# DanielaCourel/smoothed_particle_hydrodynamics

Measured on AMD Instinct MI355X. Metric: Mparticle-steps/sec (whole node), dam-break, higher is better.
Workload: dtype f32

## Files before the change

include/sph_hip.h:

```cpp
#ifndef SPH_HIP_H
#define SPH_HIP_H

#include <stddef.h>
#include <stdint.h>

#ifdef __cplusplus
extern "C" {
#endif

#define SPH_HIP_ABI_VERSION 7
#define SPH_HIP_ABI_DIAGNOSTIC 0x4000
int sph_hip_abi_version(void);

typedef enum sph_hip_status {
   SPH_HIP_OK = 0,
   SPH_HIP_ERR_INVALID = -1,
   SPH_HIP_ERR_DEVICE = -2,
   SPH_HIP_ERR_CAPACITY = -3,
   SPH_HIP_ERR_NO_DEVICE = -4,
   SPH_HIP_ERR_EXCHANGE = -5
} sph_hip_status;

typedef enum sph_hip_mode {
   SPH_HIP_MODE_REF = 0,
// ... 42 lines not shown
#define SPH_HIP_MIN_EXAMINE_COUNT 4
int sph_hip_create(sph_hip_context** out, const sph_hip_params* params, int capacity, int mode,
                   int device);
void sph_hip_destroy(sph_hip_context* ctx);

const char* sph_hip_last_error(const sph_hip_context* ctx);

int sph_hip_set_params(sph_hip_context* ctx, const sph_hip_params* params);
int sph_hip_get_params(const sph_hip_context* ctx, sph_hip_params* out);

#define SPH_HIP_ARITH_EXACT 0
#define SPH_HIP_ARITH_FAST 1
int sph_hip_set_arithmetic(sph_hip_context* ctx, int arithmetic);
int sph_hip_get_arithmetic(const sph_hip_context* ctx);


int sph_hip_upload(sph_hip_context* ctx, int n, const float* pos, const float* vel,
                   const float* mass);

int sph_hip_download(sph_hip_context* ctx, float* pos, float* vel, float* density, float* acc,
                     int32_t* neighbor_count);

int sph_hip_download_async(sph_hip_context* ctx, float* pos, float* vel, float* density, float* acc,
                           int32_t* neighbor_count, int32_t* voxel_counts, int* started);
int sph_hip_download_done(sph_hip_context* ctx, int wait);
int sph_hip_host_register(void* ptr, size_t bytes);
int sph_hip_host_unregister(void* ptr);

int sph_hip_particle_count(const sph_hip_context* ctx);


int sph_hip_step(sph_hip_context* ctx);
int sph_hip_run(sph_hip_context* ctx, int steps);

int sph_hip_voxelize(sph_hip_context* ctx);
int sph_hip_find_neighbors(sph_hip_context* ctx);
int sph_hip_compute_density(sph_hip_context* ctx);
int sph_hip_compute_acceleration(sph_hip_context* ctx);
int sph_hip_integrate(sph_hip_context* ctx);

int sph_hip_synchronize(sph_hip_context* ctx);


int sph_hip_get_timings(sph_hip_context* ctx, float ms[6]);
int sph_hip_get_phase_totals(sph_hip_context* ctx, double ms[6], int32_t* steps);
int sph_hip_reset_timings(sph_hip_context* ctx);
#define SPH_HIP_TIMING_OFF 0
#define SPH_HIP_TIMING_SUMS 1
#define SPH_HIP_TIMING_PHASES 2
int sph_hip_set_timing(sph_hip_context* ctx, int level);
int sph_hip_set_timing_stride(sph_hip_context* ctx, int every);

int sph_hip_get_tile_stats(sph_hip_context* ctx, int32_t out[20]);

int sph_hip_get_energy(sph_hip_context* ctx, float* kinetic, float* potential);

int sph_hip_get_neighbor_stats(sph_hip_context* ctx, int32_t* avg, int32_t* max, int32_t* min);

int sph_hip_download_voxels(sph_hip_context* ctx, int32_t* coords_xyz, int32_t* ids);
int sph_hip_download_grid_counts(sph_hip_context* ctx, int32_t* counts);
int sph_hip_download_neighbor_lists(sph_hip_context* ctx, uint32_t* neighbors, float* distances);


int sph_hip_sample_points(sph_hip_context* ctx, int n, const float* xyz,
                          float* density, float* velocity_xyz, int32_t* count);
int sph_hip_sample_lattice(sph_hip_context* ctx, const float origin[3], const float spacing[3],
                           const int32_t dims[3], float* density, float* velocity_xyz, int32_t* count);

#define SPH_HIP_SURFACE_NORMALS  1
#define SPH_HIP_SURFACE_VELOCITY 2
int sph_hip_extract_surface(sph_hip_context* ctx, const float origin[3], const float spacing[3],
                            const int32_t dims[3], float iso, int flags, int32_t counts[2]);
int sph_hip_download_surface(sph_hip_context* ctx, float* vertices_xyz, float* normals_xyz,
                             float* velocity_xyz, int32_t* triangles);

typedef struct sph_hip_camera {
   float eye[3];
   float forward[3];
   float right[3];
   float up[3];
} sph_hip_camera;

typedef struct sph_hip_render_params {
   float box_lo[3], box_hi[3];
   float step;
   float iso;
   int32_t refine;
   float grad_step;
   float light[3];
   float albedo[3], ambient, diffuse;
   uint8_t background[4];
   int32_t max_samples;
} sph_hip_render_params;

#define SPH_HIP_RENDER_VELOCITY 1
int sph_hip_render(sph_hip_context* ctx, const sph_hip_camera* cam, const sph_hip_render_params* rp,
                   int width, int height, int flags, uint8_t* rgba, float* depth,
                   float* normal_xyz, float* velocity_xyz, int32_t* first_inside);

typedef struct sph_hip_scene_params {
   float albedo[3];
   float ambient, diffuse;
} sph_hip_scene_params;

int sph_hip_render_scene(sph_hip_context* ctx, const sph_hip_camera* cam, const sph_hip_render_params* rp,
                         const sph_hip_scene_params* sp, const float* solid_albedo_rgb ,
// ... 173 lines not shown
```

smoothed_particle_hydrodynamics_amd/csrc/full_tiled.h:

```cpp
#pragma once

#include "launch_policy.h"
#include "tile_layout.h"
#include "common_kernels.h"
#include "full_kernels.h"
#include "neighbor_lists.h"
#include "slab_kernels.h"

#if defined(SPH_ABLATE) && !defined(SPH_DIAGNOSTIC_BUILD)
#error "SPH_ABLATE is for diagnostic builds only: add -DSPH_DIAGNOSTIC_BUILD (tools/build_variant.sh does)"
#endif

#ifdef SPH_TRIPCOUNT
#ifndef SPH_DIAGNOSTIC_BUILD
#error "SPH_TRIPCOUNT is for diagnostic builds only: add -DSPH_DIAGNOSTIC_BUILD"
#endif
enum {
   TRIP_D_WAVES = 0, TRIP_D_CHUNKS_W, TRIP_D_TEST8_W, TRIP_D_TEST8_L, TRIP_D_SLOTS_L, TRIP_D_POPS_W,
   TRIP_D_POPS_L, TRIP_D_POPLOOPS_W, TRIP_D_SUMTRIPS_W, TRIP_D_SUMSLOTS_W, TRIP_D_LISTED_L, TRIP_D_LANES_L,
   TRIP_A_WAVES = 16, TRIP_A_PTRIPS_W, TRIP_A_CNT_L, TRIP_A_VTRIPS_W, TRIP_A_NV_L, TRIP_A_LANES_L,
   TRIP_COUNT = 32
};
__device__ unsigned long long g_trip[TRIP_COUNT];
struct TripCounters {
// ... 38 lines not shown

constexpr int TILE_BATCH = 8;
#define DENSITY_TILE_BYTES 12
#define ACCEL_TILE_BYTES 16
constexpr int DENSITY_BLOCKS = 6 * 256 / TILE_THREADS;
constexpr int ACCEL_BLOCKS = TILE_THREADS == 256 ? 5 : 2;
constexpr int APPEND_POPS = 4;
constexpr int VISC_UNROLL = 4;

typedef float __attribute__((ext_vector_type(2))) f32x2;
typedef float __attribute__((ext_vector_type(4))) f32x4;

__device__ __forceinline__ f32x4 lds_read4(const float* base, int i)
{
   return *reinterpret_cast<const f32x4*>(__builtin_assume_aligned(base + i, 16));
}

struct TileLds {
   float* x;
   float* y;
   float* z;
};

extern __shared__ __attribute__((aligned(16))) float tile_lds_dynamic[];

__device__ __forceinline__ void
tile_desc(int tile, int ntiles, const uint32_t* __restrict__ perm, const uint32_t* __restrict__ key,
          const uint32_t* __restrict__ cell_start, const int32_t* __restrict__ meta, CellGrid g,
          TileDesc* __restrict__ desc, const TileCaps& caps, int32_t* __restrict__ stats,
          uint32_t* __restrict__ giveup_density, uint32_t* __restrict__ giveup_accel)
{
   const int begin = meta[META_SUM_BEGIN], end = meta[META_SUM_END];
   const int p0 = begin + tile * TILE_THREADS;
   int most = -1;
   if (tile < ntiles && p0 < end) {
      const int plast = min(p0 + TILE_THREADS - 1, end - 1);
      const int c_first = (int)key[perm[p0]];
      const int c_last = (int)key[perm[plast]];
      TileDesc d;
      int G[9], len[9];
#pragma unroll
      for (int k = 0; k < 9; k++) {
         const int off = ((k / 3 - 1) * g.ny + (k % 3 - 1)) * g.nx;
         int lo = c_first + off - 1, hi = c_last + off + 1;
         lo = lo < 0 ? 0 : lo;
         hi = hi > g.ncells - 1 ? g.ncells - 1 : hi;
         G[k] = 0;
         len[k] = 0;
         if (hi >= lo) {
            G[k] = (int)cell_start[lo];
            len[k] = (int)cell_start[hi + 1] - G[k];
         }
      }
      tile_layout_chain(G, len, d);
      const int run = d.total;
      desc[tile] = d;
      most = run;
   }
   const bool lead = (threadIdx.x & (SPH_WAVE - 1)) == 0;
#pragma unroll
   for (int c = 0; c < TILE_CANDS; c++) {
      const int over = __popcll(__ballot(c < caps.n_cand && most > caps.cand[c]));
      if (lead && over) atomicAdd(&stats[TSTAT_OVER + c], over);
   }
   int wave_most = most;
#pragma unroll
   for (int o = SPH_WAVE / 2; o > 0; o >>= 1) wave_most = max(wave_most, __shfl_xor(wave_most, o));
   if (lead && wave_most > stats[TSTAT_MAX]) atomicMax(&stats[TSTAT_MAX], wave_most);
   if (most > caps.cap_density) giveup_density[atomicAdd(&stats[TSTAT_GIVEUP_DENSITY], 1)] = (uint32_t)tile;
   if (most > caps.cap_density || most > caps.cap_accel)
      giveup_accel[atomicAdd(&stats[TSTAT_GIVEUP_ACCEL], 1)] = (uint32_t)tile;
}

__global__ void __launch_bounds__(256)
k_rank_gather_tile_desc(int desc_blocks, int ntiles, const uint32_t* __restrict__ perm,
                        const uint32_t* __restrict__ key, const uint32_t* __restrict__ cell_start,
                        const int32_t* __restrict__ meta, CellGrid g,
                        const float4* __restrict__ posm_in, const float4* __restrict__ velp_in,
                        float4* __restrict__ posm_out, float4* __restrict__ velp_out,
                        TileDesc* __restrict__ desc, TileCaps caps, int32_t* __restrict__ stats,
                        uint32_t* __restrict__ giveup_density, uint32_t* __restrict__ giveup_accel,
                        uint32_t* __restrict__ remap)
{
   if ((int)blockIdx.x < desc_blocks) {
      tile_desc(blockIdx.x * blockDim.x + threadIdx.x, ntiles, perm, key, cell_start, meta, g, desc,
                caps, stats, giveup_density, giveup_accel);
      return;
   }
   __shared__ uint32_t lds_id[256];
   rank_gather((blockIdx.x - desc_blocks) * blockDim.x + threadIdx.x,
               (blockIdx.x - desc_blocks) * blockDim.x, lds_id, perm, key, cell_start, meta,
               g.ncells, posm_in, velp_in, posm_out, velp_out, remap);
}

__device__ __forceinline__ void tile_desc_load(const TileDesc* __restrict__ desc, int wg, TileDesc& sd)
{
   const int tid = threadIdx.x;
   if (tid < (int)(sizeof(TileDesc) / sizeof(int)))
      reinterpret_cast<int*>(&sd)[tid] = reinterpret_cast<const int*>(&desc[wg])[tid];
   __syncthreads();
}

__device__ __forceinline__ int xcd_workgroup(int block, int nblocks)
{
   const int q = nblocks / 8, r = nblocks % 8, x = block % 8;
   return (x < r ? x * (q + 1) : r * (q + 1) + (x - r) * q) + block / 8;
}
// ... 593 lines not shown
            to_right = near_right;
         } else if (near_left || near_right) {
            atomicOr(&fs.meta[META_ERRORS], 8);
         }
      }
      if (fs.zone.have_left) {
         const int s = msg_reserve(&fs.left->header[0], to_left);
         if (to_left) {
            if (s < fs.msg_capacity) {
               fs.left->rec[2 * s] = x;
               fs.left->rec[2 * s + 1] = v;
            } else {
               atomicOr(&fs.meta[META_ERRORS], 2);
            }
         }
      }
      if (fs.zone.have_right) {
         const int s = msg_reserve(&fs.right->header[0], to_right);
         if (to_right) {
            if (s < fs.msg_capacity) {
               fs.right->rec[2 * s] = x;
               fs.right->rec[2 * s + 1] = v;
            } else {
               atomicOr(&fs.meta[META_ERRORS], 2);
            }
         }
      }
   }
   __shared__ double s_ke[TILE_THREADS / SPH_WAVE], s_pe[TILE_THREADS / SPH_WAVE];
#pragma unroll
   for (int d = SPH_WAVE / 2; d > 0; d >>= 1) {
      ke += __shfl_down(ke, d);
      pe += __shfl_down(pe, d);
   }
   const int lane = threadIdx.x & (SPH_WAVE - 1), w = threadIdx.x / SPH_WAVE;
   if (lane == 0) {
      s_ke[w] = ke;
      s_pe[w] = pe;
   }
   __syncthreads();
   if (threadIdx.x == 0) {
      double sa = 0.0, sb = 0.0;
#pragma unroll
      for (int q = 0; q < TILE_THREADS / SPH_WAVE; q++) {
         sa += s_ke[q];
         sb += s_pe[q];
      }
      fs.epart[2 * wg_index + 0] = sa;
      fs.epart[2 * wg_index + 1] = sb;
   }
   __syncthreads();
}

template <bool UNIT_SCALE, bool UNIFORM_MASS, bool WIDE, bool FAST>
__device__ __forceinline__ float4
accel_from_lists(int p, int cnt, const ListReader& lr, const TileDesc& d,
                 const float4* __restrict__ posm, const float4* __restrict__ velB,
                 const float* __restrict__ rho, const float* __restrict__ auxc, const PairConsts& k)
{
   const float4 pi = posm[p];
   AccelState s;
   accel_begin(k, s, pi, velB[p], rho[p]);
   const bool in_range = accel_operands_in_range(k);
   int first_v = 0;
   if (FAST) first_v = visc_first(cnt, s.visc_scale);
   if constexpr (FAST) {
      const int lastb = cnt > 0 ? (cnt - 1) >> 3 : 0;
      uint4 blk = lr.block(0);
      for (int j0 = 0; j0 < cnt; j0 += 8) {
         uint32_t entry[8];
         list_block_entries(blk, entry);
         blk = lr.block(min((j0 >> 3) + 1, lastb));
         float4 pj[8];
         float cj[8];
#pragma unroll
         for (int u = 0; u < 8; u++) {
            const uint32_t e = j0 + u < cnt ? entry[u] : entry[0];
            const int q = ListEntry<WIDE>::tile(e) - ListEntry<WIDE>::shift(d, e);
            pj[u] = posm[q];
            cj[u] = auxc[q];
         }
#pragma unroll
         for (int u = 0; u < 8; u++) {
            if (j0 + u < cnt) {
               float dx, dy, dz;
               float dd = sqrt_rn(dist2(pi.x, pi.y, pi.z, pj[u].x, pj[u].y, pj[u].z, dx, dy, dz));
               if (!UNIT_SCALE) dd *= k.sim_scale;
               accel_pair_fast_pressure<UNIT_SCALE>(k, s, dx, dy, dz, dd, cj[u]);
            }
         }
      }
      for (int j0 = first_v; j0 < cnt; j0 += VISC_UNROLL) {
         float4 pj[VISC_UNROLL], vj[VISC_UNROLL];
#pragma unroll
         for (int u = 0; u < VISC_UNROLL; u++) {
            const uint32_t e = lr.entry((uint32_t)min(j0 + u, cnt - 1));
            const int q = ListEntry<WIDE>::tile(e) - ListEntry<WIDE>::shift(d, e);
            pj[u] = posm[q];
            vj[u] = velB[q];
         }
#pragma unroll
         for (int u = 0; u < VISC_UNROLL; u++) {
            if (j0 + u < cnt) {
               float dx, dy, dz;
               float dd = sqrt_rn(dist2(pi.x, pi.y, pi.z, pj[u].x, pj[u].y, pj[u].z, dx, dy, dz));
               if (!UNIT_SCALE) dd *= k.sim_scale;
// ... 24 lines not shown
            float dx, dy, dz;
            const float d2 = dist2(pi.x, pi.y, pi.z, pj[u].x, pj[u].y, pj[u].z, dx, dy, dz);
            float dd = sqrt_rn(d2);
            if (!UNIT_SCALE) dd *= k.sim_scale;
            if (FAST) {
               accel_pair_fast_pressure<UNIT_SCALE>(k, s, dx, dy, dz, dd, cj[u]);
               if (j0 + u >= first_v) accel_pair_fast_viscous(k, s, dd, vj[u].x, vj[u].y, vj[u].z, vj[u].w);
            } else {
               accel_pair<UNIT_SCALE>(k, s, dx, dy, dz, dd, UNIFORM_MASS ? pi.w : pj[u].w, vj[u].x, vj[u].y,
                                      vj[u].z, vj[u].w, cj[u], in_range);
            }
         }
      }
   }
   if (FAST) accel_fast_finish(k, s);
   return accel_end<UNIT_SCALE>(k, s);
}

template <bool UNIT_SCALE, bool UNIFORM_MASS, bool WIDE, bool FAST>
__global__ void __launch_bounds__(TILE_THREADS, ACCEL_BLOCKS)
k_full_accel_lists(const float4* __restrict__ posm, const float4* __restrict__ velB,
                   const float* __restrict__ rho, const float* __restrict__ auxc,
                   const int32_t* __restrict__ ncount, const uint32_t* __restrict__ cell_start,
                   const int32_t* __restrict__ meta, CellGrid g, PairConsts k,
                   float4* __restrict__ acc, const TileDesc* __restrict__ desc,
                   const uint32_t* __restrict__ nlist, const uint32_t* __restrict__ nlist_overflow,
                   int tile_cap, const int32_t* __restrict__ tile_stats,
                   const uint32_t* __restrict__ giveup, int part, int list_cap,
                   int* __restrict__ tile_feedback, FusedStep fs, int tile_cap_density)
{
   PHASE_BEGIN();
   __shared__ AccelLds L;
   float4* xyzc = reinterpret_cast<float4*>(tile_lds_dynamic);
   constexpr int BATCH = TILE_BATCH;

   const int begin = meta[META_SUM_BEGIN], end = meta[META_SUM_END];
   const int ob = meta[META_OWN_BEGIN], oe = meta[META_OWN_END];
   const int tid = threadIdx.x;
   const int wgs = tile_stats[TSTAT_BLOCKS];
   const int mapped = accel_part_workgroup(part, blockIdx.x, wgs, begin, meta);
   const int wg = mapped < 0 ? 0 : mapped;
   const int p0 = begin + wg * TILE_THREADS;
   if (blockIdx.x == 0 && tid == 0) {
      tile_feedback[TSTAT_NO_LIST] = tile_stats[TSTAT_NO_LIST];
      if (fs.slab && part == 1) {
         if (fs.left) fs.left->header[1] = fs.msg_capacity;
         if (fs.right) fs.right->header[1] = fs.msg_capacity;
      }
   }
   const bool own = mapped >= 0 && !(p0 >= end || p0 + TILE_THREADS <= ob || p0 >= oe) &&
                    accel_part_has(part, p0, meta);
   const uint32_t gave_up = own ? nlist_overflow[wg] : LISTS_NONE;
   int desc_word = 0;
   if (tid < (int)(sizeof(TileDesc) / sizeof(int))) desc_word = reinterpret_cast<const int*>(&desc[wg])[tid];
   if ((int)blockIdx.x < tile_stats[TSTAT_GIVEUP_ACCEL]) {
      const int g0 = begin + (int)giveup[blockIdx.x] * TILE_THREADS;
      const int gp = g0 + tid;
      const bool mine = gp < end && gp >= ob && gp < oe && accel_part_has(part, g0, meta);
      const int gwg = (int)giveup[blockIdx.x];
      const uint32_t glists = nlist_overflow[gwg];
      if (glists != LISTS_NONE) {
         tile_desc_load(desc, gwg, L.desc);
         if (mine) {
            const int gcnt = ncount[gp];
            const ListReader glr(nlist, gwg, list_cap, tid);
            if (glists == LISTS_SOME && gcnt > 0 && glr.no_list())
               accel_untiled<UNIT_SCALE, FAST>(gp, posm, velB, rho, auxc, cell_start, g, k, acc, ncount);
            else
               acc[gp] = accel_from_lists<UNIT_SCALE, UNIFORM_MASS, WIDE, FAST>(gp, gcnt, glr, L.desc, posm, velB,
                                                                                rho, auxc, k);
         }
         __syncthreads();
      } else if (mine) {
         accel_untiled<UNIT_SCALE, FAST>(gp, posm, velB, rho, auxc, cell_start, g, k, acc, ncount);
      }
      if (fs.on && accel_part_has(part, g0, meta)) {
         float4 gx = make_float4(0.f, 0.f, 0.f, 0.f), ga = gx;
         if (mine) {
            gx = posm[gp];
            ga = acc[gp];
         }
         fused_integrate<UNIT_SCALE>(fs, k, g, gp, mine, gx, ga, (int)giveup[blockIdx.x]);
      }
   }
   if (gave_up == LISTS_NONE) return;
   if (tid < (int)(sizeof(TileDesc) / sizeof(int))) reinterpret_cast<int*>(&L.desc)[tid] = desc_word;
   __syncthreads();
   PHASE_MARK(16);
   const int total = L.desc.total;
   if (total > tile_cap || total > tile_cap_density) return;
   int B[9], D[9];
#pragma unroll
   for (int kk = 0; kk < 9; kk++) {
      B[kk] = L.desc.B[kk];
      D[kk] = L.desc.D[kk];
   }
   float4 buf[BATCH];
   float cbuf[BATCH];
#if defined(SPH_ABLATE) && SPH_ABLATE == 23
#pragma unroll
   for (int r = 0; r < BATCH; r++) {
      buf[r] = make_float4(0.f, 0.f, 0.f, 0.f);
      cbuf[r] = 0.f;
   }
   const int filled = 0;
#else
#pragma unroll
   for (int r = 0; r < BATCH; r++) {
      const int idx = min(tid + r * TILE_THREADS, total - 1);
      int d = D[0];
#pragma unroll
      for (int kk = 1; kk < 9; kk++) d = (idx >= B[kk]) ? D[kk] : d;
      buf[r] = posm[idx - d];
      cbuf[r] = auxc[idx - d];
   }
   const int filled = total;
#endif

   const int col = tid;
   const int p = p0 + col;
   const bool live = p < end && p >= ob && p < oe;
   float4 pi = make_float4(0.f, 0.f, 0.f, 0.f);
   float4 vi = pi;
   float rho_i = 0.0f;
   int cnt = 0;
   if (live) {
      pi = posm[p];
      vi = velB[p];
      rho_i = rho[p];
      cnt = ncount[p];
   }

   const ListReader lr(nlist, wg, list_cap, col);
   uint32_t entry[LIST_BLOCK_ENTRIES];
   uint4 next_blk = lr.block(0);

#pragma unroll
   for (int r = 0; r < BATCH; r++) {
      const int idx = tid + r * TILE_THREADS;
      if (idx < filled) xyzc[idx] = make_float4(buf[r].x, buf[r].y, buf[r].z, cbuf[r]);
   }

   AccelState s;
   int first_v = 0;
   bool no_list = false;
   float4 vpre[VISC_UNROLL];
   int tpre[VISC_UNROLL], nvp = 0;
   uint32_t ev[VISC_UNROLL];
   if constexpr (FAST) {
      static_assert(VISC_UNROLL == 4, "list_entries_from takes four entries");
      accel_begin(k, s, pi, vi, rho_i);
      first_v = visc_first(cnt, s.visc_scale);
      const int lcnt = cnt <= list_cap ? cnt : 0;
      const int fv = lcnt > 0 ? first_v : 0;
      const int lb = lcnt > 0 ? (lcnt - 1) >> 3 : 0;
      const int fb = fv >> 3;
      const uint4 blk_a = lr.block(fb), blk_b = lr.block(min(fb + 1, lb));
      if (gave_up == LISTS_SOME && cnt > 0) no_list = next_blk.x == NLIST_NO_LIST;
      nvp = no_list ? 0 : lcnt - fv;
      list_entries_from(blk_a, blk_b, (uint32_t)(fv & 7), ev);
   }

   for (int base = BATCH * TILE_THREADS; base < filled; base += BATCH * TILE_THREADS) {
#pragma unroll
      for (int r = 0; r < BATCH; r++) {
         const int idx = min(base + tid + r * TILE_THREADS, filled - 1);
         int d = D[0];
#pragma unroll
         for (int kk = 1; kk < 9; kk++) d = (idx >= B[kk]) ? D[kk] : d;
         buf[r] = posm[idx - d];
         cbuf[r] = auxc[idx - d];
      }
#pragma unroll
      for (int r = 0; r < BATCH; r++) {
         const int idx = base + tid + r * TILE_THREADS;
         if (idx < filled) xyzc[idx] = make_float4(buf[r].x, buf[r].y, buf[r].z, cbuf[r]);
      }
   }
   if constexpr (FAST) {
#pragma unroll
      for (int u = 0; u < VISC_UNROLL; u++) {
         tpre[u] = ListEntry<WIDE>::tile(ev[u]);
         vpre[u] = make_float4(0.f, 0.f, 0.f, 0.f);
         if (u < nvp) vpre[u] = velB[tpre[u] - ListEntry<WIDE>::shift(L.desc, ev[u])];
      }
   }
   __syncthreads();

   PHASE_MARK(17);
   if constexpr (!FAST) accel_begin(k, s, pi, vi, rho_i);
   const bool in_range = accel_operands_in_range(k);
   if constexpr (!FAST) {
      if (gave_up == LISTS_SOME && cnt > 0) no_list = next_blk.x == NLIST_NO_LIST;
   }
   if (no_list) cnt = 0;
#if defined(SPH_ABLATE) && (SPH_ABLATE == 21 || SPH_ABLATE == 23)
   cnt = 0;
#endif
   const int lastb = cnt > 0 ? (cnt - 1) >> 3 : 0;
   if constexpr (FAST) {
      TRIP(TripCounters trips; trips.wave(TRIP_A_WAVES - 16, true); trips.lane(TRIP_A_CNT_L - 16, (unsigned)cnt);
           trips.lane(TRIP_A_LANES_L - 16, live ? 1u : 0u); trips.lane(TRIP_A_NV_L - 16, (unsigned)(cnt - first_v));)
      const int nv = cnt - first_v;
      if (__any(0 < nv)) {
#pragma unroll
         for (int u = 0; u < VISC_UNROLL; u++) {
            if (u < nv) {
               const float4 pj = xyzc[tpre[u]];
               float dx, dy, dz;
               float d = sqrt_rn(dist2(pi.x, pi.y, pi.z, pj.x, pj.y, pj.z, dx, dy, dz));
               if (!UNIT_SCALE) d *= k.sim_scale;
               accel_pair_fast_viscous(k, s, d, vpre[u].x, vpre[u].y, vpre[u].z, vpre[u].w);
            }
         }
      }
      for (int m0 = VISC_UNROLL; __any(m0 < nv); m0 += VISC_UNROLL) {
         float4 vj[VISC_UNROLL];
         int tj[VISC_UNROLL];
#pragma unroll
         for (int u = 0; u < VISC_UNROLL; u++) {
            const int j = min(first_v + m0 + u, cnt > 0 ? cnt - 1 : 0);
            const uint32_t e = lr.entry((uint32_t)j);
            tj[u] = ListEntry<WIDE>::tile(e);
            vj[u] = make_float4(0.f, 0.f, 0.f, 0.f);
            if (m0 + u < nv) vj[u] = velB[tj[u] - ListEntry<WIDE>::shift(L.desc, e)];
// ... 133 lines not shown
```

smoothed_particle_hydrodynamics_amd/csrc/sph_hip.hip:

```cpp

#include "slab_comm.h"

#ifndef M_PI
#define M_PI 3.14159265358979323846
#endif

namespace {

__global__ void k_selftest_sqrt(unsigned long long* __restrict__ out)
{
   unsigned long long bad = 0;
   uint32_t first = 0xffffffffu, last = 0u;
   const uint32_t stride = gridDim.x * blockDim.x;
   for (uint64_t b = blockIdx.x * blockDim.x + threadIdx.x; b <= 0x7f7fffffull; b += stride) {
      const float x = __uint_as_float((uint32_t)b);
      const float want = sqrtf(x), got = sqrt_rn(x);
      if (__float_as_uint(want) != __float_as_uint(got)) {
         bad++;
         first = min(first, (uint32_t)b);
         last = max(last, (uint32_t)b);
      }
   }
   if (bad) {
      atomicAdd(&out[0], bad);
// ... 1495 lines not shown

int sph_hip_reset_timings(sph_hip_context* ctx)
{
   if (!ctx) return SPH_HIP_ERR_INVALID;
   ctx->ev_steps = 0;
   return SPH_HIP_OK;
}

int sph_hip_get_phase_totals(sph_hip_context* ctx, double ms[6], int32_t* steps)
{
   int rc = check_ctx(ctx);
   if (rc) return rc;
   if (!ms || !steps) return SPH_HIP_ERR_INVALID;
   const long long have = ctx->ev_steps < EV_RING ? ctx->ev_steps : EV_RING;
   for (int k = 0; k < 6; k++) ms[k] = 0.0;
   for (long long s = ctx->ev_steps - have; s < ctx->ev_steps; s++) {
      float one[6];
      if ((rc = read_phases(ctx, ctx->ev[s % EV_RING], one))) return rc;
      for (int k = 0; k < 6; k++) ms[k] += (double)one[k];
   }
   *steps = (int32_t)have;
   return SPH_HIP_OK;
}

int sph_hip_get_energy(sph_hip_context* ctx, float* kinetic, float* potential)
{
   int rc = check_ctx(ctx);
   if (rc) return rc;
   double e[2] = {0.0, 0.0};
   if (ctx->energy_blocks > 0) {
      hipLaunchKernelGGL(k_energy_total, dim3(1), dim3(RED_THREADS), 0, ctx->stream,
                         ctx->epart + 2, ctx->energy_blocks, ctx->epart);
      SPH_TRY(hipGetLastError());
   }
   SPH_TRY(hipMemcpyAsync(e, ctx->epart, sizeof(e), hipMemcpyDeviceToHost, ctx->stream));
   SPH_TRY(hipStreamSynchronize(ctx->stream));
   if (kinetic) *kinetic = (float)e[0];
   if (potential) *potential = (float)e[1];
   return SPH_HIP_OK;
}

int sph_hip_get_tile_stats(sph_hip_context* ctx, int32_t out[20])
{
   int rc = check_ctx(ctx);
   if (rc) return rc;
   if (!out || !ctx->tile_feedback) return SPH_HIP_ERR_INVALID;
   SPH_TRY(hipStreamSynchronize(ctx->stream));
   for (int i = 0; i < 16; i++) out[i] = ctx->tile_feedback[i];
   out[16] = ctx->caps.cap_density;
   out[17] = ctx->caps.cap_accel;
   out[18] = ctx->caps.wide;
   out[19] = ctx->list_cap;
   return SPH_HIP_OK;
}

int sph_hip_get_neighbor_stats(sph_hip_context* ctx, int32_t* avg, int32_t* mx, int32_t* mn)
{
   int rc = check_ctx(ctx);
   if (rc) return rc;
   if ((rc = owned_count(ctx, nullptr))) return rc;
   const int n = ctx->n_owned;
   if (n == 0) return SPH_HIP_ERR_INVALID;
   const int32_t init[4] = {0, 0, -1, 34};
   SPH_TRY(hipMemcpyAsync(ctx->stats, init, sizeof(init), hipMemcpyHostToDevice, ctx->stream));
   int blocks = div_up(n, RED_THREADS);
   if (blocks > 1024) blocks = 1024;
   hipLaunchKernelGGL(k_neighbor_stats, dim3(blocks), dim3(RED_THREADS), 0, ctx->stream,
                      ctx->ncount, ctx->meta, ctx->stats);
   SPH_TRY(hipGetLastError());
   int32_t out[4];
   SPH_TRY(hipMemcpyAsync(out, ctx->stats, sizeof(out), hipMemcpyDeviceToHost, ctx->stream));
   SPH_TRY(hipStreamSynchronize(ctx->stream));
   const long long sum = ((long long)(uint32_t)out[1] << 32) | (uint32_t)out[0];
   if (avg) *avg = (int32_t)(sum / n);
   if (mx) *mx = out[2];
   if (mn) *mn = out[3];
   return SPH_HIP_OK;
}

int sph_hip_download_voxels(sph_hip_context* ctx, int32_t* coords_xyz, int32_t* ids)
{
   int rc = check_ctx(ctx);
   if (rc) return rc;
   if (ctx->mode != SPH_HIP_MODE_REF) {
      ctx->err = "sph_hip_download_voxels: REF-mode contexts only";
      return SPH_HIP_ERR_INVALID;
   }
   const int n = ctx->n_owned;
   if (coords_xyz)
      SPH_TRY(hipMemcpyAsync(coords_xyz, ctx->vox, sizeof(int32_t) * 3 * n, hipMemcpyDeviceToHost,
                             ctx->stream));
   if (ids)
      SPH_TRY(hipMemcpyAsync(ids, ctx->key, sizeof(int32_t) * n, hipMemcpyDeviceToHost, ctx->stream));
   SPH_TRY(hipStreamSynchronize(ctx->stream));
   return SPH_HIP_OK;
}

int sph_hip_download_grid_counts(sph_hip_context* ctx, int32_t* counts)
{
   int rc = check_ctx(ctx);
   if (rc) return rc;
   if (!counts) return SPH_HIP_ERR_INVALID;
   const int nc = ctx->grid.ncells;
   uint32_t* tmp = (uint32_t*)malloc(sizeof(uint32_t) * ((size_t)nc + 1));
   if (!tmp) return SPH_HIP_ERR_INVALID;
   hipError_t e = hipMemcpyAsync(tmp, ctx->cell_start, sizeof(uint32_t) * ((size_t)nc + 1),
// ... 578 lines not shown
```

smoothed_particle_hydrodynamics_amd/csrc/tile_layout.h:

```cpp
#pragma once

#include <stdint.h>

#include "launch_policy.h"

#ifdef __HIPCC__
#define TILE_HD __host__ __device__ inline __attribute__((always_inline))
#else
#define TILE_HD inline
#endif

#define TILE_SEGMENTS 9
#define TILE_EACH_BOUNDARY(X) X(1, 0) X(2, 1) X(3, 2) X(4, 3) X(5, 4) X(6, 5) X(7, 6) X(8, 7)
#define TILE_WORDS(k, prev) const int B##k = B[k], D##k = D[k];
#define TILE_LOCALS const int D0 = D[0]; TILE_EACH_BOUNDARY(TILE_WORDS)

struct TileDesc {
   int D[9];
   int B[9];
   int total;
   int pad;
};

TILE_HD void tile_layout_chain(const int (&G)[TILE_SEGMENTS], const int (&len)[TILE_SEGMENTS], TileDesc& d)
{
   int run = 0, chain_end = -1, chain_d = 0;
#ifdef __HIPCC__
#pragma unroll
#endif
   for (int k = 0; k < TILE_SEGMENTS; k++) {
      d.B[k] = run;
      if (len[k] == 0) {
         d.D[k] = run - G[k];
      } else if (G[k] <= chain_end) {
         const int seg_end = G[k] + len[k];
         d.D[k] = chain_d;
         if (seg_end > chain_end) {
            run += seg_end - chain_end;
            chain_end = seg_end;
         }
      } else {
         d.D[k] = chain_d = run - G[k];
         run += len[k];
         chain_end = G[k] + len[k];
      }
   }
   d.total = run;
   d.pad = 0;
}

TILE_HD int tile_shift_at(const int (&B)[TILE_SEGMENTS], const int (&D)[TILE_SEGMENTS], int t)
{
   TILE_LOCALS
   int d = D0;
#define TILE_STEP(k, prev) d = (t >= B##k) ? D##k : d;
   TILE_EACH_BOUNDARY(TILE_STEP)
#undef TILE_STEP
   return d;
}

TILE_HD uint32_t tile_pass_boundaries(const int (&B)[TILE_SEGMENTS], const int (&D)[TILE_SEGMENTS], int lo, int hi)
{
   TILE_LOCALS
   uint32_t m = 0;
#define TILE_STEP(k, prev) m |= ((B##k > lo) & (B##k < hi) & (D##k != D##prev)) ? 1u << k : 0u;
   TILE_EACH_BOUNDARY(TILE_STEP)
#undef TILE_STEP
   return m;
}

TILE_HD uint64_t tile_pass_mask(const int (&B)[TILE_SEGMENTS], const int (&D)[TILE_SEGMENTS], int total)
{
   TILE_LOCALS
   uint64_t m = 0;
#define TILE_STEP(k, prev)                                                                          \
   m |= ((B##k > 0) & (B##k < total) & (B##k % TILE_THREADS != 0) & (D##k != D##prev))             \
           ? 1ull << (B##k / TILE_THREADS < 63 ? B##k / TILE_THREADS : 63) : 0ull;
   TILE_EACH_BOUNDARY(TILE_STEP)
#undef TILE_STEP
   return m;
}
TILE_HD bool tile_pass_has_boundary(uint64_t mask, int q)
{
   return (mask >> (q < 63 ? q : 63)) & 1u;
}

struct TilePassPlan {
   int first, end;
   int shift;
   int n;
   int B[TILE_SEGMENTS - 1];
   int D[TILE_SEGMENTS - 1];
};
TILE_HD void tile_pass_plan(const TileDesc& d, int q, TilePassPlan& p)
{
   p.first = q * TILE_THREADS;
   p.end = p.first + TILE_THREADS < d.total ? p.first + TILE_THREADS : d.total;
   if (p.end < p.first) p.end = p.first;
   p.shift = tile_shift_at(d.B, d.D, p.first);
   p.n = 0;
   if (!tile_pass_has_boundary(tile_pass_mask(d.B, d.D, d.total), q)) return;
   const uint32_t m = tile_pass_boundaries(d.B, d.D, p.first, p.end);
   for (int k = 1; k < TILE_SEGMENTS; k++)
      if (m >> k & 1u) {
         p.B[p.n] = d.B[k];
         p.D[p.n] = d.D[k];
         p.n++;
      }
}
```

smoothed_particle_hydrodynamics_amd/lib.py:

```python
import collections
import ctypes as C
import os

from .build import library_path

MODE_REF = 0
MODE_FULL = 1
MODE_FULL_FAST = 2
ARITH_EXACT, ARITH_FAST = 0, 1
ABI_DIAGNOSTIC = 0x4000
TIMING_OFF, TIMING_SUMS, TIMING_PHASES = 0, 1, 2


class SphHipError(RuntimeError):
    pass


class SphParams(C.Structure):

    _fields_ = [
        ("cells_x", C.c_int32), ("cells_y", C.c_int32), ("cells_z", C.c_int32),
        ("cell_size", C.c_float),
        ("max_x", C.c_float), ("max_y", C.c_float), ("max_z", C.c_float),
        ("h", C.c_float), ("h2", C.c_float), ("hscaled", C.c_float), ("hscaled2", C.c_float),
# ... 35 lines not shown

    _fields_ = [
        ("box_lo", C.c_float * 3), ("box_hi", C.c_float * 3),
        ("step", C.c_float), ("iso", C.c_float), ("refine", C.c_int32), ("grad_step", C.c_float),
        ("light", C.c_float * 3), ("albedo", C.c_float * 3), ("ambient", C.c_float), ("diffuse", C.c_float),
        ("background", C.c_uint8 * 4), ("max_samples", C.c_int32),
    ]


class SphSceneParams(C.Structure):

    _fields_ = [("albedo", C.c_float * 3), ("ambient", C.c_float), ("diffuse", C.c_float)]


from . import obstacles as _obstacles
from .obstacles import (SphBody, SphBodyState, SphMotionKey, SphMotionPath, SphObstacle,
                        SphObstacleMotion)
from .gauges import GaugeReadings, GaugeRecord, SphGauge
from .ports import PortTotals, SphEmitter, SphSink

_P = C.POINTER
_ctx = C.c_void_p
PROTOTYPES = {
    "sph_hip_params_default": (C.c_int, [_P(SphParams), C.c_float, C.c_int, C.c_int, C.c_int]),
    "sph_hip_create": (C.c_int, [_P(_ctx), _P(SphParams), C.c_int, C.c_int, C.c_int]),
    "sph_hip_destroy": (None, [_ctx]),
    "sph_hip_last_error": (C.c_char_p, [_ctx]),
    "sph_hip_set_params": (C.c_int, [_ctx, _P(SphParams)]),
    "sph_hip_get_params": (C.c_int, [_ctx, _P(SphParams)]),
    "sph_hip_set_arithmetic": (C.c_int, [_ctx, C.c_int]),
    "sph_hip_get_arithmetic": (C.c_int, [_ctx]),
    "sph_hip_upload": (C.c_int, [_ctx, C.c_int, C.c_void_p, C.c_void_p, C.c_void_p]),
    "sph_hip_download": (C.c_int, [_ctx, C.c_void_p, C.c_void_p, C.c_void_p, C.c_void_p, C.c_void_p]),
    "sph_hip_particle_count": (C.c_int, [_ctx]),
    "sph_hip_download_async": (C.c_int, [_ctx, C.c_void_p, C.c_void_p, C.c_void_p, C.c_void_p,
                                         C.c_void_p, C.c_void_p, _P(C.c_int)]),
    "sph_hip_download_done": (C.c_int, [_ctx, C.c_int]),
    "sph_hip_host_register": (C.c_int, [C.c_void_p, C.c_size_t]),
    "sph_hip_host_unregister": (C.c_int, [C.c_void_p]),
    "sph_hip_step": (C.c_int, [_ctx]),
    "sph_hip_run": (C.c_int, [_ctx, C.c_int]),
    "sph_hip_voxelize": (C.c_int, [_ctx]),
    "sph_hip_find_neighbors": (C.c_int, [_ctx]),
    "sph_hip_compute_density": (C.c_int, [_ctx]),
    "sph_hip_compute_acceleration": (C.c_int, [_ctx]),
    "sph_hip_integrate": (C.c_int, [_ctx]),
    "sph_hip_synchronize": (C.c_int, [_ctx]),
    "sph_hip_get_timings": (C.c_int, [_ctx, _P(C.c_float * 6)]),
    "sph_hip_get_phase_totals": (C.c_int, [_ctx, _P(C.c_double * 6), _P(C.c_int32)]),
    "sph_hip_reset_timings": (C.c_int, [_ctx]),
    "sph_hip_set_timing": (C.c_int, [_ctx, C.c_int]),
    "sph_hip_set_timing_stride": (C.c_int, [_ctx, C.c_int]),
    "sph_hip_get_tile_stats": (C.c_int, [_ctx, _P(C.c_int32 * 20)]),
    "sph_hip_get_energy": (C.c_int, [_ctx, _P(C.c_float), _P(C.c_float)]),
    "sph_hip_get_neighbor_stats": (C.c_int, [_ctx, _P(C.c_int32), _P(C.c_int32), _P(C.c_int32)]),
    "sph_hip_download_voxels": (C.c_int, [_ctx, C.c_void_p, C.c_void_p]),
    "sph_hip_download_grid_counts": (C.c_int, [_ctx, C.c_void_p]),
    "sph_hip_download_neighbor_lists": (C.c_int, [_ctx, C.c_void_p, C.c_void_p]),
    "sph_hip_sample_points": (C.c_int, [_ctx, C.c_int, C.c_void_p, C.c_void_p, C.c_void_p, C.c_void_p]),
    "sph_hip_sample_pressure_points": (C.c_int, [_ctx, C.c_int, C.c_void_p, C.c_void_p, C.c_void_p, C.c_void_p]),
    "sph_hip_sample_pressure_lattice": (C.c_int, [_ctx, _P(C.c_float * 3), _P(C.c_float * 3), _P(C.c_int32 * 3),
                                                  C.c_void_p, C.c_void_p, C.c_void_p]),
    "sph_hip_sample_lattice": (C.c_int, [_ctx, _P(C.c_float * 3), _P(C.c_float * 3), _P(C.c_int32 * 3),
                                         C.c_void_p, C.c_void_p, C.c_void_p]),
    "sph_hip_extract_surface": (C.c_int, [_ctx, _P(C.c_float * 3), _P(C.c_float * 3), _P(C.c_int32 * 3), C.c_float,
                                          C.c_int, _P(C.c_int32 * 2)]),
    "sph_hip_download_surface": (C.c_int, [_ctx, C.c_void_p, C.c_void_p, C.c_void_p, C.c_void_p]),
    "sph_hip_render": (C.c_int, [_ctx, _P(SphCamera), _P(SphRenderParams), C.c_int, C.c_int, C.c_int,
                                 C.c_void_p, C.c_void_p, C.c_void_p, C.c_void_p, C.c_void_p]),
    "sph_hip_render_scene": (C.c_int, [_ctx, _P(SphCamera), _P(SphRenderParams), _P(SphSceneParams), C.c_void_p,
                                       C.c_int, C.c_int, C.c_int, C.c_int, C.c_void_p, C.c_void_p, C.c_void_p,
                                       C.c_void_p, C.c_void_p, C.c_void_p]),
    "sph_hip_set_obstacles": (C.c_int, [_ctx, _P(SphObstacle), C.c_int]),
    "sph_hip_get_obstacles": (C.c_int, [_ctx, _P(SphObstacle), C.c_int]),
    "sph_hip_set_obstacle_motion": (C.c_int, [_ctx, _P(SphObstacleMotion), C.c_int]),
    "sph_hip_get_obstacle_motion": (C.c_int, [_ctx, _P(SphObstacleMotion), C.c_int, _P(C.c_float)]),
    "sph_hip_get_obstacles_now": (C.c_int, [_ctx, _P(SphObstacle), C.c_int]),
    "sph_hip_set_obstacle_paths": (C.c_int, [_ctx, _P(SphMotionPath), C.c_int, _P(SphMotionKey), C.c_int]),
    "sph_hip_get_obstacle_paths": (C.c_int, [_ctx, _P(SphMotionPath), C.c_int, _P(SphMotionKey), C.c_int,
                                             C.c_void_p]),
    "sph_hip_set_bodies": (C.c_int, [_ctx, _P(SphBody), C.c_int, C.c_int]),
    "sph_hip_get_bodies": (C.c_int, [_ctx, _P(SphBody), _P(SphBodyState), C.c_int]),
    "sph_hip_record_loads": (C.c_int, [_ctx, C.c_int, C.c_int]),
    "sph_hip_get_loads": (C.c_int, [_ctx, C.c_int, C.c_int, C.c_void_p, C.c_void_p, C.c_void_p, _P(C.c_int32)]),
    "sph_hip_set_tracers": (C.c_int, [_ctx, C.c_int, C.c_void_p]),
    "sph_hip_get_tracers": (C.c_int, [_ctx, C.c_int, C.c_int, C.c_void_p, C.c_void_p, C.c_void_p]),
    "sph_hip_tracer_count": (C.c_int, [_ctx]),
    "sph_hip_record_tracers": (C.c_int, [_ctx, C.c_int, C.c_int]),
    "sph_hip_get_tracer_path": (C.c_int, [_ctx, C.c_int, C.c_int, C.c_void_p, C.c_void_p]),
    "sph_hip_set_gauges": (C.c_int, [_ctx, _P(SphGauge), C.c_int]),
    "sph_hip_get_gauges": (C.c_int, [_ctx, _P(SphGauge), C.c_int]),
    "sph_hip_read_gauges": (C.c_int, [_ctx, C.c_void_p]),
    "sph_hip_record_gauges": (C.c_int, [_ctx, C.c_int, C.c_int]),
    "sph_hip_get_gauge_record": (C.c_int, [_ctx, C.c_int, C.c_int, C.c_void_p, C.c_void_p]),
    "sph_hip_set_ports": (C.c_int, [_ctx, _P(SphEmitter), C.c_int, _P(SphSink), C.c_int]),
    "sph_hip_get_ports": (C.c_int, [_ctx, _P(SphEmitter), _P(SphSink), C.c_int, C.c_int, C.c_void_p, C.c_void_p,
                                    _P(C.c_int32), _P(C.c_uint32)]),
    "sph_hip_download_live": (C.c_int, [_ctx, C.c_int, _P(C.c_int32), C.c_void_p, C.c_void_p, C.c_void_p, C.c_void_p,
                                        C.c_void_p, C.c_void_p]),
    "sph_hip_stream": (C.c_void_p, [_ctx]),
    "sph_hip_set_stream": (C.c_int, [_ctx, C.c_void_p]),
    "sph_hip_create_slab": (C.c_int, [_P(_ctx), _P(SphParams), C.c_int, C.c_int, C.c_int, C.c_int]),
    "sph_hip_slab_upload": (C.c_int, [_ctx, C.c_int, C.c_void_p, C.c_void_p, C.c_void_p,
                                      C.c_void_p, C.c_int]),
    "sph_hip_slab_download": (C.c_int, [_ctx, C.c_int, _P(C.c_int32), C.c_void_p, C.c_void_p,
                                        C.c_void_p, C.c_void_p, C.c_void_p, C.c_void_p]),
# ... 103 lines not shown
TracerPath = collections.namedtuple("TracerPath", ["steps", "positions"])


class Context:

    def __init__(self, creator, *args):
        self._lib = load_library()
        self._ctx = C.c_void_p()
        rc = getattr(self._lib, creator)(C.byref(self._ctx), *args)
        if rc != 0:
            msg = self._lib.sph_hip_last_error(None).decode()
            self._ctx = C.c_void_p()
            raise SphHipError("%s failed (%d): %s" % (creator, rc, msg))

    def close(self):
        if getattr(self, "_ctx", None) is not None and self._ctx:
            self._lib.sph_hip_destroy(self._ctx)
            self._ctx = C.c_void_p()

    def __del__(self):
        try:
            self.close()
        except Exception:
            pass

    def __enter__(self):
        return self

    def __exit__(self, *exc):
        self.close()

    def call(self, name, *args):
        fn = getattr(self._lib, name)
        return self.check(fn, fn(self._ctx, *args))

    def check(self, fn, rc):
        if rc < 0:
            msg = self._lib.sph_hip_last_error(self._ctx).decode()
            raise SphHipError("%s failed (%d): %s" % (fn.__name__, rc, msg))
        return rc

    def synchronize(self):
        self.call("sph_hip_synchronize")

    def tile_stats(self):
        out = (C.c_int32 * 20)()
        self.call("sph_hip_get_tile_stats", C.byref(out))
        v = list(out)
        return {"over_level": v[0:12], "workgroups": v[12], "largest_tile": v[13],
                "untiled_density": v[14], "untiled_acceleration": v[15],
                "capacity_density": v[16], "capacity_acceleration": v[17], "wide_entries": v[18],
                "list_capacity": v[19]}

    def phase_totals(self):
        ms = (C.c_double * 6)()
        k = C.c_int32()
        self.call("sph_hip_get_phase_totals", C.byref(ms), C.byref(k))
        return list(ms), k.value

    def energy(self):
        ke, pe = C.c_float(), C.c_float()
        self.call("sph_hip_get_energy", C.byref(ke), C.byref(pe))
        return ke.value, pe.value

    def reset_timings(self):
        self.call("sph_hip_reset_timings")

    def set_timing(self, level):
        self.call("sph_hip_set_timing", int(level))

    def set_timing_stride(self, every):
        self.call("sph_hip_set_timing_stride", int(every))

    def set_arithmetic(self, arithmetic):
        self.call("sph_hip_set_arithmetic", int(arithmetic))

    def set_obstacles(self, obstacles):
        arr, n = _obstacles.as_array(obstacles)
        self.call("sph_hip_set_obstacles", arr, n)

    def get_obstacles(self, now=False):
        arr = (SphObstacle * _obstacles.MAX_OBSTACLES)()
        n = self.call("sph_hip_get_obstacles_now" if now else "sph_hip_get_obstacles", arr, _obstacles.MAX_OBSTACLES)
        return [_obstacles.from_struct(arr[i]) for i in range(n)]

    def set_obstacle_motion(self, motions):
        arr, n = _obstacles.as_motion_array(motions)
        self.call("sph_hip_set_obstacle_motion", arr, n)

    def get_obstacle_motion(self):
        arr = (SphObstacleMotion * _obstacles.MAX_OBSTACLES)()
        clock = C.c_float()
        n = self.call("sph_hip_get_obstacle_motion", arr, _obstacles.MAX_OBSTACLES, C.byref(clock))
        return [_obstacles.motion_from_struct(arr[i]) for i in range(n)], clock.value

    def set_obstacle_paths(self, paths):
        arr, n, keys, n_keys = _obstacles.as_path_arrays(paths)
        self.call("sph_hip_set_obstacle_paths", arr, n, keys, n_keys)

    def get_obstacle_paths(self, shifts=True):
        import numpy as np
        arr = (SphMotionPath * _obstacles.MAX_OBSTACLES)()
        keys = (SphMotionKey * _obstacles.MAX_PATH_KEYS)()
        out = np.zeros((_obstacles.MAX_OBSTACLES, 2, 3), np.float32)
        n = self.call("sph_hip_get_obstacle_paths", arr, _obstacles.MAX_OBSTACLES, keys, _obstacles.MAX_PATH_KEYS,
                      _ptr(out) if shifts else None)
# ... 30 lines not shown
```

smoothed_particle_hydrodynamics_amd/sph.py:

```python
import collections
import ctypes as C
import math
import struct
import zlib

import numpy as np

from . import gauges as _G
from . import obstacles as _O
from . import ports as _P
from .lib import ARITH_EXACT, ARITH_FAST, MODE_FULL, MODE_FULL_FAST, MODE_REF, Bodies, Context, SphCamera, SphRenderParams, SphSceneParams, TracerPath, Tracers, _ptr, default_params

__all__ = ["SPH", "Particle", "SurfaceMesh", "Tracers", "TracerPath", "Camera", "RenderResult", "write_png", "MODE_REF", "MODE_FULL", "MODE_FULL_FAST", "ARITH_EXACT", "ARITH_FAST"]


class Particle:

    def __init__(self, num_particles):
        n = int(num_particles)
        self.mMass = np.zeros(n, np.float32)
        self.mDensity = np.zeros(n, np.float32)
        self.mPosition = np.zeros(3 * n, np.float32)
        self.mVelocity = np.zeros(3 * n, np.float32)
        self.mAcceleration = np.zeros(3 * n, np.float32)
# ... 429 lines not shown
        rp.box_lo[:] = [float(v) for v in np.asarray(box[0], f).reshape(3)]
        rp.box_hi[:] = [float(v) for v in np.asarray(box[1], f).reshape(3)]
        rp.step = float(f(0.5) * h) if step is None else float(step)
        rp.iso = float(iso)
        rp.refine = int(refine)
        rp.grad_step = float(f(0.5) * h) if grad_step is None else float(grad_step)
        rp.light[:] = [float(v) for v in light]
        rp.albedo[:] = [float(v) for v in albedo]
        rp.ambient = float(ambient)
        rp.diffuse = float(diffuse)
        rp.background[:] = [int(v) for v in background]
        rp.max_samples = int(max_samples)
        return rp

    def render(self, camera, width, height, iso, step=None, refine=8, grad_step=None, box=None,
               light=(0.4, 0.8, 0.45), albedo=(0.25, 0.55, 0.9), ambient=0.2, diffuse=0.8,
               background=(0, 0, 0, 255), velocity=False, max_samples=1 << 16, solids=False,
               solid_albedo=(0.72, 0.72, 0.72), solid_colors=None, solid_ambient=None, solid_diffuse=None):
        rp = self.renderParams(iso, step, refine, grad_step, box, light, albedo, ambient, diffuse, background,
                               max_samples)
        W, H = int(width), int(height)
        if W < 1 or H < 1:
            raise ValueError("width and height must be positive")
        rgba = np.zeros((H, W, 4), np.uint8)
        depth = np.zeros((H, W), np.float32)
        normal = np.zeros((H, W, 3), np.float32)
        vel = np.zeros((H, W, 3), np.float32) if velocity else None
        first = np.zeros((H, W), np.int32)
        cam = camera.as_struct()
        flags = RENDER_VELOCITY if velocity else 0
        if not solids:
            self.call("sph_hip_render", C.byref(cam), C.byref(rp), W, H, flags,
                      _ptr(rgba), _ptr(depth), _ptr(normal), _ptr(vel), _ptr(first))
            return RenderResult(rgba, depth, normal, vel, first)
        sp = SphSceneParams()
        sp.albedo[:] = [float(v) for v in solid_albedo]
        sp.ambient = float(ambient if solid_ambient is None else solid_ambient)
        sp.diffuse = float(diffuse if solid_diffuse is None else solid_diffuse)
        colors = None if solid_colors is None else np.ascontiguousarray(solid_colors, np.float32).reshape(-1, 3)
        solid_id = np.zeros((H, W), np.int32)
        self.call("sph_hip_render_scene", C.byref(cam), C.byref(rp), C.byref(sp), _ptr(colors),
                  0 if colors is None else colors.shape[0], W, H, flags,
                  _ptr(rgba), _ptr(depth), _ptr(normal), _ptr(vel), _ptr(first), _ptr(solid_id))
        return RenderResult(rgba, depth, normal, vel, first, solid_id)

    def elapsed(self):
        ms = (C.c_float * 6)()
        self.call("sph_hip_get_timings", C.byref(ms))
        return list(ms)

    resetTimings, setTiming = Context.reset_timings, Context.set_timing
    setTimingStride = Context.set_timing_stride
    tileStats, phaseTotals = Context.tile_stats, Context.phase_totals

    def neighborStats(self):
        a, b, c = C.c_int32(), C.c_int32(), C.c_int32()
        self.call("sph_hip_get_neighbor_stats", C.byref(a), C.byref(b), C.byref(c))
        return a.value, b.value, c.value

    def voxels(self):
        n = self.mParticleCount
        coords = np.zeros(3 * n, np.int32)
        ids = np.zeros(n, np.int32)
        self.call("sph_hip_download_voxels", _ptr(coords), _ptr(ids))
        return coords, ids

    def neighborLists(self):
        m = self.mParticleCount * self._params.examine_count
        nb = np.zeros(m, np.uint32)
        nd = np.zeros(m, np.float32)
        self.call("sph_hip_download_neighbor_lists", _ptr(nb), _ptr(nd))
        return nb, nd


def write_ply(path, mesh):
    v = np.ascontiguousarray(mesh.vertices, np.float32).reshape(-1, 3)
    t = np.ascontiguousarray(mesh.triangles, np.int32).reshape(-1, 3)
    n = getattr(mesh, "normals", None)
    fields = [("x", "<f4"), ("y", "<f4"), ("z", "<f4")]
    if n is not None:
        fields += [("nx", "<f4"), ("ny", "<f4"), ("nz", "<f4")]
    vert = np.empty(len(v), dtype=fields)
    vert["x"], vert["y"], vert["z"] = v[:, 0], v[:, 1], v[:, 2]
    if n is not None:
        n = np.asarray(n, np.float32).reshape(-1, 3)
        vert["nx"], vert["ny"], vert["nz"] = n[:, 0], n[:, 1], n[:, 2]
    face = np.empty(len(t), dtype=[("n", "u1"), ("i", "<i4", (3,))])
    face["n"] = 3
    face["i"] = t
    head = ["ply", "format binary_little_endian 1.0", "element vertex %d" % len(v)]
    head += ["property float %s" % name for name, _ in fields]
    head += ["element face %d" % len(t), "property list uchar int vertex_indices", "end_header"]
    with open(path, "wb") as f:
        f.write(("\n".join(head) + "\n").encode("ascii"))
        f.write(vert.tobytes())
        f.write(face.tobytes())


def write_png(path, rgba):
    img = np.ascontiguousarray(rgba, np.uint8)
    if img.ndim != 3 or img.shape[2] != 4:
        raise ValueError("rgba must be (H, W, 4) uint8")
    H, W = img.shape[0], img.shape[1]
    raw = np.concatenate([np.zeros((H, 1), np.uint8), img.reshape(H, W * 4)], 1).tobytes()

    def chunk(tag, data):
# ... 8 lines not shown
```

Baseline: 4931.

## Precompute tile chain summary and prefetch short-chain tiles before barrier

```diff
diff --git a/include/sph_hip.h b/include/sph_hip.h
--- a/include/sph_hip.h
+++ b/include/sph_hip.h
@@ -118,6 +118,7 @@
 int sph_hip_set_timing_stride(sph_hip_context* ctx, int every);
 
 int sph_hip_get_tile_stats(sph_hip_context* ctx, int32_t out[20]);
+int sph_hip_get_tile_descriptors(sph_hip_context* ctx, int32_t* out, int max_workgroups);
 
 int sph_hip_get_energy(sph_hip_context* ctx, float* kinetic, float* potential);
 
diff --git a/smoothed_particle_hydrodynamics_amd/csrc/full_tiled.h b/smoothed_particle_hydrodynamics_amd/csrc/full_tiled.h
--- a/smoothed_particle_hydrodynamics_amd/csrc/full_tiled.h
+++ b/smoothed_particle_hydrodynamics_amd/csrc/full_tiled.h
@@ -114,7 +114,7 @@
             len[k] = (int)cell_start[hi + 1] - G[k];
          }
       }
-      tile_layout_chain(G, len, d);
+      tile_layout_describe(G, len, d);
       const int run = d.total;
       desc[tile] = d;
       most = run;
@@ -814,6 +814,45 @@
    __syncthreads();
 }
 
+__device__ __forceinline__ void accel_fill_short(const float4* __restrict__ posm, const float* __restrict__ auxc,
+                                                 int D0, int BA, int DA, int BB, int DB, int base, int last,
+                                                 float4 (&buf)[TILE_BATCH], float (&cbuf)[TILE_BATCH])
+{
+   const int tid = threadIdx.x;
+#pragma unroll
+   for (int r = 0; r < TILE_BATCH; r++) {
+      const int idx = min(base + tid + r * TILE_THREADS, last);
+      const int d = tile_shift_short(D0, BA, DA, BB, DB, idx);
+      buf[r] = posm[idx - d];
+      cbuf[r] = auxc[idx - d];
+   }
+}
+__device__ __forceinline__ void accel_fill_batch(const float4* __restrict__ posm, const float* __restrict__ auxc,
+                                                 const TileDesc& sd, bool few, int ka, int kb, int base, int last,
+                                                 float4 (&buf)[TILE_BATCH], float (&cbuf)[TILE_BATCH])
+{
+   const int tid = threadIdx.x;
+   if (few) {
+      accel_fill_short(posm, auxc, sd.D[0], sd.B[ka], sd.D[ka], sd.B[kb], sd.D[kb], base, last, buf, cbuf);
+   } else {
+      int B[9], D[9];
+#pragma unroll
+      for (int kk = 0; kk < 9; kk++) {
+         B[kk] = sd.B[kk];
+         D[kk] = sd.D[kk];
+      }
+#pragma unroll
+      for (int r = 0; r < TILE_BATCH; r++) {
+         const int idx = min(base + tid + r * TILE_THREADS, last);
+         int d = D[0];
+#pragma unroll
+         for (int kk = 1; kk < 9; kk++) d = (idx >= B[kk]) ? D[kk] : d;
+         buf[r] = posm[idx - d];
+         cbuf[r] = auxc[idx - d];
+      }
+   }
+}
+
 template <bool UNIT_SCALE, bool UNIFORM_MASS, bool WIDE, bool FAST>
 __device__ __forceinline__ float4
 accel_from_lists(int p, int cnt, const ListReader& lr, const TileDesc& d,
@@ -944,7 +983,8 @@
                     accel_part_has(part, p0, meta);
    const uint32_t gave_up = own ? nlist_overflow[wg] : LISTS_NONE;
    int desc_word = 0;
-   if (tid < (int)(sizeof(TileDesc) / sizeof(int))) desc_word = reinterpret_cast<const int*>(&desc[wg])[tid];
+   const int desc_lane = tid & (SPH_WAVE - 1);
+   if (desc_lane < (int)(sizeof(TileDesc) / sizeof(int))) desc_word = reinterpret_cast<const int*>(&desc[wg])[desc_lane];
    if ((int)blockIdx.x < tile_stats[TSTAT_GIVEUP_ACCEL]) {
       const int g0 = begin + (int)giveup[blockIdx.x] * TILE_THREADS;
       const int gp = g0 + tid;
@@ -976,19 +1016,26 @@
       }
    }
    if (gave_up == LISTS_NONE) return;
+   const int chains = __builtin_amdgcn_readlane(desc_word, (int)(offsetof(TileDesc, pad) / sizeof(int)));
+   const bool few_chains = tile_chains_short(chains);
+   const int chain_ka = tile_chains_ka(chains), chain_kb = tile_chains_kb(chains);
+   float4 buf[BATCH];
+   float cbuf[BATCH];
+#if !(defined(SPH_ABLATE) && SPH_ABLATE == 23)
+   if (few_chains) {
+      constexpr int WD = (int)(offsetof(TileDesc, D) / sizeof(int)), WB = (int)(offsetof(TileDesc, B) / sizeof(int));
+      const int wave_total = __builtin_amdgcn_readlane(desc_word, (int)(offsetof(TileDesc, total) / sizeof(int)));
+      accel_fill_short(posm, auxc, __builtin_amdgcn_readlane(desc_word, WD),
+                       __builtin_amdgcn_readlane(desc_word, WB + chain_ka), __builtin_amdgcn_readlane(desc_word, WD + chain_ka),
+                       __builtin_amdgcn_readlane(desc_word, WB + chain_kb), __builtin_amdgcn_readlane(desc_word, WD + chain_kb),
+                       0, wave_total - 1, buf, cbuf);
+   }
+#endif
    if (tid < (int)(sizeof(TileDesc) / sizeof(int))) reinterpret_cast<int*>(&L.desc)[tid] = desc_word;
    __syncthreads();
    PHASE_MARK(16);
    const int total = L.desc.total;
    if (total > tile_cap || total > tile_cap_density) return;
-   int B[9], D[9];
-#pragma unroll
-   for (int kk = 0; kk < 9; kk++) {
-      B[kk] = L.desc.B[kk];
-      D[kk] = L.desc.D[kk];
-   }
-   float4 buf[BATCH];
-   float cbuf[BATCH];
 #if defined(SPH_ABLATE) && SPH_ABLATE == 23
 #pragma unroll
    for (int r = 0; r < BATCH; r++) {
@@ -997,15 +1044,7 @@
    }
    const int filled = 0;
 #else
-#pragma unroll
-   for (int r = 0; r < BATCH; r++) {
-      const int idx = min(tid + r * TILE_THREADS, total - 1);
-      int d = D[0];
-#pragma unroll
-      for (int kk = 1; kk < 9; kk++) d = (idx >= B[kk]) ? D[kk] : d;
-      buf[r] = posm[idx - d];
-      cbuf[r] = auxc[idx - d];
-   }
+   if (!few_chains) accel_fill_batch(posm, auxc, L.desc, false, 0, 0, 0, total - 1, buf, cbuf);
    const int filled = total;
 #endif
 
@@ -1054,15 +1093,7 @@
    }
 
    for (int base = BATCH * TILE_THREADS; base < filled; base += BATCH * TILE_THREADS) {
-#pragma unroll
-      for (int r = 0; r < BATCH; r++) {
-         const int idx = min(base + tid + r * TILE_THREADS, filled - 1);
-         int d = D[0];
-#pragma unroll
-         for (int kk = 1; kk < 9; kk++) d = (idx >= B[kk]) ? D[kk] : d;
-         buf[r] = posm[idx - d];
-         cbuf[r] = auxc[idx - d];
-      }
+      accel_fill_batch(posm, auxc, L.desc, few_chains, chain_ka, chain_kb, base, filled - 1, buf, cbuf);
 #pragma unroll
       for (int r = 0; r < BATCH; r++) {
          const int idx = base + tid + r * TILE_THREADS;
diff --git a/smoothed_particle_hydrodynamics_amd/csrc/sph_hip.hip b/smoothed_particle_hydrodynamics_amd/csrc/sph_hip.hip
--- a/smoothed_particle_hydrodynamics_amd/csrc/sph_hip.hip
+++ b/smoothed_particle_hydrodynamics_amd/csrc/sph_hip.hip
@@ -1571,6 +1571,20 @@
    out[18] = ctx->caps.wide;
    out[19] = ctx->list_cap;
    return SPH_HIP_OK;
+}
+
+int sph_hip_get_tile_descriptors(sph_hip_context* ctx, int32_t* out, int max_workgroups)
+{
+   int rc = check_ctx(ctx);
+   if (rc) return rc;
+   if (!out || max_workgroups < 0 || !ctx->tile_feedback || !ctx->tile_desc) return SPH_HIP_ERR_INVALID;
+   SPH_TRY(hipStreamSynchronize(ctx->stream));
+   int n = ctx->tile_feedback[TSTAT_BLOCKS];
+   if (n > max_workgroups) n = max_workgroups;
+   if (n <= 0) return 0;
+   SPH_TRY(hipMemcpyAsync(out, ctx->tile_desc, (size_t)n * sizeof(TileDesc), hipMemcpyDeviceToHost, ctx->stream));
+   SPH_TRY(hipStreamSynchronize(ctx->stream));
+   return n;
 }
 
 int sph_hip_get_neighbor_stats(sph_hip_context* ctx, int32_t* avg, int32_t* mx, int32_t* mn)
diff --git a/smoothed_particle_hydrodynamics_amd/csrc/tile_layout.h b/smoothed_particle_hydrodynamics_amd/csrc/tile_layout.h
--- a/smoothed_particle_hydrodynamics_amd/csrc/tile_layout.h
+++ b/smoothed_particle_hydrodynamics_amd/csrc/tile_layout.h
@@ -49,6 +49,35 @@
    d.pad = 0;
 }
 
+#define TILE_CHAINS_SHORT 3
+TILE_HD int tile_chains_n(int word) { return word & 15; }
+TILE_HD int tile_chains_ka(int word) { return (word >> 4) & 15; }
+TILE_HD int tile_chains_kb(int word) { return (word >> 8) & 15; }
+TILE_HD bool tile_chains_short(int word) { return (unsigned)(tile_chains_n(word) - 1) < (unsigned)TILE_CHAINS_SHORT; }
+TILE_HD int tile_chain_word(const int (&B)[TILE_SEGMENTS], const int (&D)[TILE_SEGMENTS], int total)
+{
+   int cur = D[0], nch = 1, ka = 0, kb = 0;
+#ifdef __HIPCC__
+#pragma unroll
+#endif
+   for (int k = 1; k < TILE_SEGMENTS; k++) {
+      const int next = k + 1 < TILE_SEGMENTS ? B[k + 1] : total;
+      if (next > B[k] && D[k] != cur) {
+         cur = D[k];
+         ka = kb;
+         kb = k;
+         nch++;
+      }
+   }
+   if (nch > TILE_CHAINS_SHORT) ka = kb = 0;
+   return nch | ka << 4 | kb << 8;
+}
+TILE_HD void tile_layout_describe(const int (&G)[TILE_SEGMENTS], const int (&len)[TILE_SEGMENTS], TileDesc& d)
+{
+   tile_layout_chain(G, len, d);
+   d.pad = tile_chain_word(d.B, d.D, d.total);
+}
+
 TILE_HD int tile_shift_at(const int (&B)[TILE_SEGMENTS], const int (&D)[TILE_SEGMENTS], int t)
 {
    TILE_LOCALS
@@ -56,6 +85,14 @@
 #define TILE_STEP(k, prev) d = (t >= B##k) ? D##k : d;
    TILE_EACH_BOUNDARY(TILE_STEP)
 #undef TILE_STEP
+   return d;
+}
+
+TILE_HD int tile_shift_short(int D0, int BA, int DA, int BB, int DB, int t)
+{
+   int d = D0;
+   d = (t >= BA) ? DA : d;
+   d = (t >= BB) ? DB : d;
    return d;
 }
 
diff --git a/smoothed_particle_hydrodynamics_amd/lib.py b/smoothed_particle_hydrodynamics_amd/lib.py
--- a/smoothed_particle_hydrodynamics_amd/lib.py
+++ b/smoothed_particle_hydrodynamics_amd/lib.py
@@ -111,6 +111,7 @@
     "sph_hip_set_timing": (C.c_int, [_ctx, C.c_int]),
     "sph_hip_set_timing_stride": (C.c_int, [_ctx, C.c_int]),
     "sph_hip_get_tile_stats": (C.c_int, [_ctx, _P(C.c_int32 * 20)]),
+    "sph_hip_get_tile_descriptors": (C.c_int, [_ctx, C.c_void_p, C.c_int]),
     "sph_hip_get_energy": (C.c_int, [_ctx, _P(C.c_float), _P(C.c_float)]),
     "sph_hip_get_neighbor_stats": (C.c_int, [_ctx, _P(C.c_int32), _P(C.c_int32), _P(C.c_int32)]),
     "sph_hip_download_voxels": (C.c_int, [_ctx, C.c_void_p, C.c_void_p]),
@@ -320,6 +321,12 @@
                 "capacity_density": v[16], "capacity_acceleration": v[17], "wide_entries": v[18],
                 "list_capacity": v[19]}
 
+    def tile_descriptors(self):
+        import numpy as np
+        rows = self.tile_stats()["workgroups"]
+        out = np.zeros((max(rows, 1), 20), np.int32)
+        return out[:self.call("sph_hip_get_tile_descriptors", _ptr(out), rows)]
+
     def phase_totals(self):
         ms = (C.c_double * 6)()
         k = C.c_int32()
diff --git a/smoothed_particle_hydrodynamics_amd/sph.py b/smoothed_particle_hydrodynamics_amd/sph.py
--- a/smoothed_particle_hydrodynamics_amd/sph.py
+++ b/smoothed_particle_hydrodynamics_amd/sph.py
@@ -505,6 +505,7 @@
     resetTimings, setTiming = Context.reset_timings, Context.set_timing
     setTimingStride = Context.set_timing_stride
     tileStats, phaseTotals = Context.tile_stats, Context.phase_totals
+    tileDescriptors = Context.tile_descriptors
 
     def neighborStats(self):
         a, b, c = C.c_int32(), C.c_int32(), C.c_int32()
```

Measured after the change: 4942 (median of 6 runs). About the same (+0.2%).
